# quentinll/pertrenderer

Hardware: NVIDIA B200
Metric: perturbed shader fwd+bwd pixel·face·samples/sec (higher is better)
Workload: dtype f32

## Files before the change

### pertrenderer_b200/csrc/tile.cuh

```cuda
#pragma once
#include "common.cuh"
#include "philox.cuh"

namespace pert {

__device__ __forceinline__ int scan_valid(const int64_t* __restrict__ p2f , int E, bool vec_ok,
                                          uint16_t* vlist, int cap) {
    const int lane = threadIdx.x & 31;
    const unsigned lt = (1u << lane) - 1u;
    int total = 0;
    constexpr int U = 4;
    for (int base = 0; base < E; base += 64 * U) {
        long long a[U], b[U];
#pragma unroll
        for (int u = 0; u < U; ++u) {
            const int e0 = base + u * 64 + 2 * lane;
            a[u] = -1;
            b[u] = -1;
            if (e0 + 1 < E) {
                if (vec_ok) {
                    const longlong2 v = __ldg(reinterpret_cast<const longlong2*>(p2f + e0));
                    a[u] = v.x;
                    b[u] = v.y;
                } else {
                    a[u] = __ldg(p2f + e0);
                    b[u] = __ldg(p2f + e0 + 1);
                }
            } else if (e0 < E) {
                a[u] = __ldg(p2f + e0);
            }
        }
#pragma unroll
        for (int u = 0; u < U; ++u) {
            if (base + u * 64 >= E) break;
            const int e0 = base + u * 64 + 2 * lane;
            const bool v0 = a[u] >= 0, v1 = b[u] >= 0;
            const unsigned be = __ballot_sync(FULL, v0), bo = __ballot_sync(FULL, v1);
            const int pos = total + __popc(be & lt) + __popc(bo & lt);
            if (v0 && pos < cap) vlist[pos] = (uint16_t)e0;
            if (v1 && pos + (v0 ? 1 : 0) < cap) vlist[pos + (v0 ? 1 : 0)] = (uint16_t)(e0 + 1);
            total += __popc(be) + __popc(bo);
        }
    }
    return total;
}

__device__ __forceinline__ unsigned smem_u32(const void* p) { return (unsigned)__cvta_generic_to_shared(p); }
__device__ __forceinline__ void mbar_init(uint64_t* bar, int count) {
    asm volatile("mbarrier.init.shared::cta.b64 [%0], %1;" ::"r"(smem_u32(bar)), "r"(count) : "memory");
    asm volatile("fence.mbarrier_init.release.cluster;" ::: "memory");
}
__device__ __forceinline__ void bulk_load(void* smem_dst, const void* gsrc, unsigned bytes, uint64_t* bar) {
    asm volatile("mbarrier.arrive.expect_tx.shared::cta.b64 _, [%0], %1;" ::"r"(smem_u32(bar)), "r"(bytes) : "memory");
    asm volatile("cp.async.bulk.shared::cluster.global.mbarrier::complete_tx::bytes [%0], [%1], %2, [%3];" ::"r"(smem_u32(smem_dst)),
                 "l"(gsrc), "r"(bytes), "r"(smem_u32(bar))
                 : "memory");
}
__device__ __forceinline__ void mbar_wait(uint64_t* bar, unsigned parity) {
    unsigned ok = 0;
#pragma unroll 1
    while (!ok) {
        asm volatile("{\n .reg .pred p;\n mbarrier.try_wait.parity.shared::cta.b64 p, [%1], %2;\n selp.u32 %0, 1, 0, p;\n}"
                     : "=r"(ok)
                     : "r"(smem_u32(bar)), "r"(parity)
                     : "memory");
    }
}

__device__ __forceinline__ int scan_valid_staged(const int64_t* __restrict__ p2f, int E, long long* stage, uint64_t* bar,
                                                 uint16_t* vlist, int cap) {
    const int lane = threadIdx.x & 31;
    const unsigned lt = (1u << lane) - 1u;
    unsigned* const par = reinterpret_cast<unsigned*>(bar + 1);
    const unsigned parity = *par;
    __syncwarp();
    if (lane == 0) {
        bulk_load(stage, p2f, (unsigned)E * 8u, bar);
        *par = parity ^ 1u;
    }
    mbar_wait(bar, parity);
    int total = 0;
#pragma unroll 1
    for (int base = 0; base < E; base += 64) {
        const int e0 = base + 2 * lane;
        long long a = -1, b = -1;
        if (e0 + 1 < E) {
            const longlong2 v = *reinterpret_cast<const longlong2*>(stage + e0);
            a = v.x;
            b = v.y;
        } else if (e0 < E) {
            a = stage[e0];
        }
        const bool v0 = a >= 0, v1 = b >= 0;
        const unsigned be = __ballot_sync(FULL, v0), bo = __ballot_sync(FULL, v1);
        const int pos = total + __popc(be & lt) + __popc(bo & lt);
        if (v0 && pos < cap) vlist[pos] = (uint16_t)e0;
        if (v1 && pos + (v0 ? 1 : 0) < cap) vlist[pos + (v0 ? 1 : 0)] = (uint16_t)(e0 + 1);
        total += __popc(be) + __popc(bo);
    }
    return total;
}

__device__ __forceinline__ void pixel_ranges(const uint16_t* vlist, int nv, int K, int tp, int* vstart) {
    const int lane = threadIdx.x & 31;
#pragma unroll 1
    for (int p = lane; p <= tp; p += 32) {
        vstart[p] = lower_bound_u16(vlist, 0, nv, p * K);
    }
}

template <class NoiseT, int SCORE = 0, bool WOVR = false, bool RENDER = false>
__device__ __forceinline__ void rast_sample_list(const NoiseT& noise, const uint16_t* rlist, int nlist,
                                                 const uint16_t* vlist, const float* xs, uint16_t* cnt, float* rs,
                                                 int K, float invK, int64_t pix0, float sigma, float inv_sigma,
                                                 int s_begin, int s_end, bool gate_ok,
                                                 int lpe_max ) {
    const int lane = threadIdx.x & 31;
    const int qb = s_begin >> 2, qe = (s_end + 3) >> 2;
    if (nlist == 0) return;
    const int lpe_shift = min(31 - __clz(lpe_max), fill_shift(nlist));
    const int lpe = 1 << lpe_shift;
    const int gpw = 32 >> lpe_shift;
    const int lig = lane & (lpe - 1);
#pragma unroll 1
    for (int base = 0; base < nlist; base += gpw) {
        const int li = base + (lane >> lpe_shift);
        const bool active = li < nlist;
        const int n = active ? rlist[li] : 0;
        const int e = vlist[n];
        const int pix = entry_pixel(e, invK), k = e - pix * K;
        const float x = xs[n];
        const bool h0 = x >= 0.0f;
        int c = 0;
        float r = 0.0f;
        if (active) {
            if constexpr (NoiseT::kBounded) {
                const uint32_t gate = (gate_ok && !(WOVR && h0)) ? radius_gate(fabsf(x) * inv_sigma * 0.99999f) : 0u;
#pragma unroll 1
                for (int q = qb + lig; q < qe; q += lpe) {
                    uint32_t w[4];
                    noise.words(q, k, pix0 + pix, w);
#pragma unroll
                    for (int hp = 0; hp < 2; ++hp) {
                        const int s0 = q * 4 + hp * 2;
                        const bool in0 = s0 >= s_begin && s0 < s_end, in1 = s0 + 1 >= s_begin && s0 + 1 < s_end;
                        if ((w[hp * 2] >> 9) < gate) {
                            if (h0) c += (in0 ? 1 : 0) + (in1 ? 1 : 0);
                        } else {
                            float n0, n1;
                            box_muller(w[hp * 2], w[hp * 2 + 1], n0, n1);
                            const bool ha = __fadd_rn(x, __fmul_rn(sigma, n0)) >= 0.0f;
                            const bool hb = __fadd_rn(x, __fmul_rn(sigma, n1)) >= 0.0f;
                            if constexpr (RENDER) {
                                c += (in0 && ha ? 1 : 0) + (in1 && hb ? 1 : 0);
                            } else if constexpr (WOVR) {
                                if (in0) {
                                    c += ha ? 1 : 0;
                                    if (ha) r += n0;
                                }
                                if (in1) {
                                    c += hb ? 1 : 0;
                                    if (hb) r += n1;
                                }
                            } else {
                                if (in0) {
                                    c += ha ? 1 : 0;
                                    if (ha != h0) r += ha ? n0 : -n0;
                                }
                                if (in1) {
                                    c += hb ? 1 : 0;
                                    if (hb != h0) r += hb ? n1 : -n1;
                                }
                            }
                        }
                    }
                }
            } else {
#pragma unroll 1
                for (int q = qb + lig; q < qe; q += lpe) {
                    float nz[4];
                    noise.get4(q, k, pix0 + pix, nz);
#pragma unroll
                    for (int t = 0; t < 4; ++t) {
                        const int s = q * 4 + t;
                        const bool h = __fadd_rn(x, __fmul_rn(sigma, nz[t])) >= 0.0f;
                        if (s >= s_begin && s < s_end) {
                            c += h ? 1 : 0;
                            if constexpr (RENDER) {
                            } else if constexpr (WOVR) {
                                if (h) r += noise_score<SCORE>(nz[t]);
                            } else if (h != h0) {
                                r += h ? noise_score<SCORE>(nz[t]) : -noise_score<SCORE>(nz[t]);
                            }
                        }
                    }
                }
            }
        }
#pragma unroll 1
        for (int o = lpe >> 1; o > 0; o >>= 1) {
            c += __shfl_xor_sync(FULL, c, o);
            if constexpr (!RENDER) r += __shfl_xor_sync(FULL, r, o);
        }
        if (active && lig == 0) {
            cnt[n] = (uint16_t)c;
            if constexpr (!RENDER) rs[n] = r;
        }
    }
}

template <class NoiseT>
struct CompoundCtx {
    NoiseT noise;
    const uint16_t* vlist;
    const float* xs;
    uint16_t* cnt;
    float* rs;
    int K;
    float invK;
    int64_t pix0;
    float inv_sigma;
    int n_loc;
    uint32_t c0;
};

template <class NoiseT>
__device__ __forceinline__ int compound_flips(const CompoundCtx<NoiseT>& c, int k, int pix, float x, uint32_t (&w)[4],
                                              float& p, float& t) {
    t = fabsf(x) * c.inv_sigma;
    p = 0.5f * erfcf(t * 0.70710678118654752f);
    const float fn = (float)c.n_loc;
    const float nl = fn * log1pf(-p);
    const float sf1 = -expm1f(nl);
    c.noise.words(c.c0, (uint32_t)k, c.pix0 + pix, w);
    const float u = ((float)w[0] + 1.0f) * 2.3283064365386963e-10f;
    int F = 0;
    if (u <= sf1) {
        float pmf = __expf(nl), sf = sf1;
        const float ratio = __fdividef(p, 1.0f - p);
        do {
            ++F;
            pmf *= ratio * __fdividef((float)(c.n_loc - F + 1), (float)F);
            sf -= pmf;
        } while (u <= sf && F < c.n_loc && (pmf > 1e-10f || (float)F < fn * p));
    }
    return F;
}

template <class NoiseT>
static __device__ __noinline__ void compound_entry(const CompoundCtx<NoiseT>& c, int n) {
    const int e = c.vlist[n];
    const int pix = entry_pixel(e, c.invK), k = e - pix * c.K;
    const float x = c.xs[n];
    uint32_t w[4];
    float p, t;
    const int F = compound_flips(c, k, pix, x, w, p, t);
    float r = 0.0f;
    if (F > 0) {
        uint32_t q = c.c0;
        int idx = 1;
#pragma unroll 1
        for (int i = 0; i < F; ++i) {
            if (idx == 4) {
                ++q;
                c.noise.words(q, (uint32_t)k, c.pix0 + pix, w);
                idx = 0;
            }
            const uint32_t word = idx == 0 ? w[0] : idx == 1 ? w[1] : idx == 2 ? w[2] : w[3];
            ++idx;
            const float v = ((float)word + 1.0f) * 2.3283064365386963e-10f;
            r += fmaxf(1.4142135623730951f * erfcinvf(2.0f * v * p), t);
        }
    }
    c.cnt[n] = (uint16_t)((x >= 0.0f) ? c.n_loc - F : F);
    c.rs[n] = r;
}

template <class NoiseT>
static __device__ __noinline__ void compound_count_entry(const CompoundCtx<NoiseT>& c, int n) {
    const int e = c.vlist[n];
    const int pix = entry_pixel(e, c.invK), k = e - pix * c.K;
    const float x = c.xs[n];
    uint32_t w[4];
    float p, t;
    const int F = compound_flips(c, k, pix, x, w, p, t);
    c.cnt[n] = (uint16_t)((x >= 0.0f) ? c.n_loc - F : F);
}

template <class NoiseT, void (*ENTRY)(const CompoundCtx<NoiseT>&, int)>
__device__ __forceinline__ void compound_sweep(const CompoundCtx<NoiseT>& c, const uint16_t* blist, int nb, float x_b2,
                                               float x_b3, uint16_t* ring) {
    const int lane = threadIdx.x & 31;
    const unsigned lt = (1u << lane) - 1u;
    if (nb <= 32) {
        if (lane < nb) ENTRY(c, blist[-lane]);
        return;
    }
#pragma unroll 1
    for (int b = 0; b < 3; ++b) {
        int have = 0, done = 0;
#pragma unroll 1
        for (int base = 0; base < nb; base += 32) {
            const int li = base + lane;
            const int n = li < nb ? blist[-li] : 0;
            const float ax = fabsf(c.xs[n]);
            const bool sel = li < nb && (ax < x_b2 ? 0 : ax < x_b3 ? 1 : 2) == b;
            const unsigned m = __ballot_sync(FULL, sel);
            if (sel) ring[(have + __popc(m & lt)) & 63] = (uint16_t)n;
            have += __popc(m);
            __syncwarp();
            if (have - done >= 32) {
                ENTRY(c, ring[(done + lane) & 63]);
                done += 32;
                __syncwarp();
            }
        }
        if (lane < have - done) ENTRY(c, ring[(done + lane) & 63]);
        __syncwarp();
    }
}

template <class NoiseT>
static __device__ __noinline__ void rast_compound_list(const CompoundCtx<NoiseT>& c, const uint16_t* blist, int nb, float x_b2,
                                                       float x_b3, uint16_t* ring) {
    compound_sweep<NoiseT, compound_entry<NoiseT>>(c, blist, nb, x_b2, x_b3, ring);
}

template <class NoiseT>
static __device__ __noinline__ void rast_compound_count_list(const CompoundCtx<NoiseT>& c, const uint16_t* blist, int nb,
                                                             float x_b2, float x_b3, uint16_t* ring) {
    compound_sweep<NoiseT, compound_count_entry<NoiseT>>(c, blist, nb, x_b2, x_b3, ring);
}

struct PixPrep {
    float zmax;
    float zimax;
    float prod_nz;
    float zeta_max;
    float zbg;
    int argzi;
    int nzero;
    int a0;
    int kpad;
};

__device__ __forceinline__ PixPrep prep_pixels(int p, int lig, int G, bool pvalid, int K, const int* vstart,
                                               const uint16_t* vlist, const uint16_t* cnt, float* zs, float zn,
                                               float zf, int S_rast, float gal, float eps) {
    const int vs = pvalid ? vstart[p] : 0, ve = pvalid ? vstart[p + 1] : 0;
    const int nv = ve - vs;
    const int e_base = p * K;
    float zimax = -CUDART_INF_F;
    int argzi = 0x7fffffff;
    float prod = 1.0f;
    int nzero = 0;
    int kpad = 0x7fffffff;
    const float denom = zf - zn;
    const float fS = (float)S_rast;
#pragma unroll 1
    for (int n = vs + lig; n < ve; n += G) {
        const int k = (int)vlist[n] - e_base;
        const float pk = (float)cnt[n] / fS;
        const float om = 1.0f - pk;
        if (om == 0.0f) nzero++; else prod *= om;
        const float zi = __fdiv_rn(zf - zs[n], denom);
        zs[n] = zi;
        if (zi > zimax) {
            zimax = zi;
            argzi = k;
        }
        if (k != n - vs) kpad = min(kpad, n - vs);
    }
    __syncwarp();
    group_argmax(zimax, argzi, G);
    prod = group_prod(prod, G);
    nzero = group_sum_i(nzero, G);
    kpad = group_min_i(kpad, G);
    if (kpad == 0x7fffffff) kpad = nv;
    if (kpad < K) {
        if (0.0f > zimax || (0.0f == zimax && kpad < argzi)) {
            zimax = 0.0f;
            argzi = kpad;
        }
    }
    const float zmax = fmaxf(zimax, eps);
    const float zbg = __fadd_rn(eps, -zmax);
    float best = -CUDART_INF_F;
    int a0 = 0x7fffffff;
#pragma unroll 1
    for (int n = vs + lig; n < ve; n += G) {
        const int k = (int)vlist[n] - e_base;
        const int c = cnt[n];
        float z = -CUDART_INF_F;
        if (c != 0) {
            const float lg = (c == S_rast) ? 0.0f : logf_exact((float)c / fS);
            z = __fadd_rn(__fadd_rn(__fmul_rn(gal, lg), zs[n]), -zmax);
        }
        zs[n] = z;
        if (z > best) {
            best = z;
            a0 = k;
        }
    }
    __syncwarp();
    group_argmax(best, a0, G);
    if (!(best >= zbg)) {
        best = zbg;
        a0 = K;
    }
    PixPrep pi;
    pi.zmax = zmax;
    pi.zimax = zimax;
    pi.prod_nz = prod;
    pi.nzero = nzero;
    pi.argzi = argzi;
    pi.a0 = a0;
    pi.zeta_max = best;
    pi.zbg = zbg;
    pi.kpad = kpad;
    return pi;
}

__device__ __forceinline__ float live_cut(float gamma, float zeta_max, bool bounded) {
    return bounded ? 2.0f * gamma * kNoiseAbsMax * 1.0001f + 4e-7f * fmaxf(1.0f, fabsf(zeta_max)) : CUDART_INF_F;
}

}
```

Baseline: 993.7 billion.

## Split compound tail sampling into head pass and flip-count-bucketed tail passes

```diff
diff --git a/pertrenderer_b200/csrc/tile.cuh b/pertrenderer_b200/csrc/tile.cuh
--- a/pertrenderer_b200/csrc/tile.cuh
+++ b/pertrenderer_b200/csrc/tile.cuh
@@ -247,8 +247,13 @@
     return F;
 }
 
-template <class NoiseT>
-static __device__ __noinline__ void compound_entry(const CompoundCtx<NoiseT>& c, int n) {
+__device__ __forceinline__ float compound_tail(uint32_t word, float p, float t) {
+    const float v = ((float)word + 1.0f) * 2.3283064365386963e-10f;
+    return fmaxf(1.4142135623730951f * erfcinvf(2.0f * v * p), t);
+}
+
+template <class NoiseT>
+static __device__ __noinline__ void compound_head_entry(const CompoundCtx<NoiseT>& c, int n) {
     const int e = c.vlist[n];
     const int pix = entry_pixel(e, c.invK), k = e - pix * c.K;
     const float x = c.xs[n];
@@ -256,23 +261,35 @@
     float p, t;
     const int F = compound_flips(c, k, pix, x, w, p, t);
     float r = 0.0f;
-    if (F > 0) {
-        uint32_t q = c.c0;
-        int idx = 1;
-#pragma unroll 1
-        for (int i = 0; i < F; ++i) {
-            if (idx == 4) {
-                ++q;
-                c.noise.words(q, (uint32_t)k, c.pix0 + pix, w);
-                idx = 0;
-            }
-            const uint32_t word = idx == 0 ? w[0] : idx == 1 ? w[1] : idx == 2 ? w[2] : w[3];
-            ++idx;
-            const float v = ((float)word + 1.0f) * 2.3283064365386963e-10f;
-            r += fmaxf(1.4142135623730951f * erfcinvf(2.0f * v * p), t);
-        }
-    }
+    const int f3 = min(F, 3);
+#pragma unroll 1
+    for (int i = 0; i < f3; ++i) r += compound_tail(i == 0 ? w[1] : i == 1 ? w[2] : w[3], p, t);
     c.cnt[n] = (uint16_t)((x >= 0.0f) ? c.n_loc - F : F);
+    c.rs[n] = r;
+}
+
+template <class NoiseT>
+__device__ __forceinline__ int compound_saved_flips(const CompoundCtx<NoiseT>& c, int n) {
+    const int cn = c.cnt[n];
+    return c.xs[n] >= 0.0f ? c.n_loc - cn : cn;
+}
+
+template <class NoiseT>
+static __device__ __noinline__ void compound_tail_entry(const CompoundCtx<NoiseT>& c, int n) {
+    const int e = c.vlist[n];
+    const int pix = entry_pixel(e, c.invK), k = e - pix * c.K;
+    const float t = fabsf(c.xs[n]) * c.inv_sigma;
+    const float p = 0.5f * erfcf(t * 0.70710678118654752f);
+    const int F = compound_saved_flips(c, n);
+    float r = c.rs[n];
+    uint32_t w[4];
+    uint32_t q = c.c0;
+#pragma unroll 1
+    for (int i = 3; i < F; ++i) {
+        const int idx = (i + 1) & 3;
+        if (idx == 0) c.noise.words(++q, (uint32_t)k, c.pix0 + pix, w);
+        r += compound_tail(idx == 0 ? w[0] : idx == 1 ? w[1] : idx == 2 ? w[2] : w[3], p, t);
+    }
     c.rs[n] = r;
 }
 
@@ -323,7 +340,31 @@
 template <class NoiseT>
 static __device__ __noinline__ void rast_compound_list(const CompoundCtx<NoiseT>& c, const uint16_t* blist, int nb, float x_b2,
                                                        float x_b3, uint16_t* ring) {
-    compound_sweep<NoiseT, compound_entry<NoiseT>>(c, blist, nb, x_b2, x_b3, ring);
+    compound_sweep<NoiseT, compound_head_entry<NoiseT>>(c, blist, nb, x_b2, x_b3, ring);
+    const int lane = threadIdx.x & 31;
+    const unsigned lt = (1u << lane) - 1u;
+#pragma unroll 1
+    for (int b = 0; b < 3; ++b) {
+        int have = 0, done = 0;
+#pragma unroll 1
+        for (int base = 0; base < nb; base += 32) {
+            const int li = base + lane;
+            const int n = li < nb ? blist[-li] : 0;
+            const int F = compound_saved_flips(c, n);
+            const bool sel = li < nb && F >= 4 && (F < 8 ? 0 : F < 16 ? 1 : 2) == b;
+            const unsigned m = __ballot_sync(FULL, sel);
+            if (sel) ring[(have + __popc(m & lt)) & 63] = (uint16_t)n;
+            have += __popc(m);
+            __syncwarp();
+            if (have - done >= 32) {
+                compound_tail_entry(c, ring[(done + lane) & 63]);
+                done += 32;
+                __syncwarp();
+            }
+        }
+        if (lane < have - done) compound_tail_entry(c, ring[(done + lane) & 63]);
+        __syncwarp();
+    }
 }
 
 template <class NoiseT>
```

Measured after the change: 968.9 billion, median of 6. 2.5% lower.
